# leggedrobotics/raisimLib

Hardware: AMD Instinct MI355X
Metric: env-steps/sec, 4096 ANYmal-C envs flat terrain dt=0.0025 (higher is better)
Workload: dtype f32

## Files before the change

raisimlib_amd/csrc/step_phase_delassus.inc:

```
      const int npw = ncw * (ncw + 1) / 2;
      for (int p0 = 0; p0 < npw; p0 += LPE) {
        const int p = p0 + s;
        const int j = (int)((__builtin_sqrtf(8.0f * (float)p + 1.5f) - 1.0f) * 0.5f);
        const int i = p - ((j * (j + 1)) >> 1);
        if (j < nc) {
          const int bi = __float_as_int(CON[i * kConSlot + 7]), bj = __float_as_int(CON[j * kConSlot + 7]);
          const int li = PARLV[bi] >> 8, lj = PARLV[bj] >> 8;
          int ai[ML], aj[ML];
#if defined(RSB_SPECIALIZED) && RSB_SPEC_DEPTH == 4
          {
            const int4 ri = *reinterpret_cast<const int4*>(ANC + bi * 4), rj = *reinterpret_cast<const int4*>(ANC + bj * 4);
            const int vi[4] = {ri.y, ri.z, ri.w, -1}, vj[4] = {rj.y, rj.z, rj.w, -2};
            RSB_UNROLL for (int l = 0; l < ML; ++l) {
              ai[l] = (l + 1 <= li && l < 3) ? vi[l < 3 ? l : 3] : -1;
              aj[l] = (l + 1 <= lj && l < 3) ? vj[l < 3 ? l : 3] : -2;
            }
          }
#else
          RSB_UNROLL for (int l = 0; l < ML; ++l) {
            ai[l] = (l + 1 <= li) ? ANC[bi * depth + l + 1] : -1;
            aj[l] = (l + 1 <= lj) ? ANC[bj * depth + l + 1] : -2;
          }
#endif
          int lca = 0;
          bool same = true;
          RSB_UNROLL for (int l = 0; l < ML; ++l) { same = same && (ai[l] == aj[l]); lca += same ? 1 : 0; }
          constexpr int CWC = 6 + ML;
          float wi[3][CWC], wj[3][CWC];
          const float* Wi = WC + (3 * i) * cw;
          const float* Wj = WC + (3 * j) * cw;
          RSB_UNROLL for (int rr = 0; rr < 3; ++rr) {
            RSB_UNROLL for (int q4 = 0; q4 < (CWC + 3) / 4; ++q4) {
              float t4[4], u4[4];
              ld4(Wi + rr * cw + 4 * q4, t4); ld4(Wj + rr * cw + 4 * q4, u4);
              RSB_UNROLL for (int e = 0; e < 4; ++e)
                if (4 * q4 + e < CWC) { wi[rr][4 * q4 + e] = t4[e]; wj[rr][4 * q4 + e] = u4[e]; }
            }
          }
          float acc[9];
          RSB_UNROLL for (int q2 = 0; q2 < 9; ++q2) acc[q2] = 0.f;
          RSB_UNROLL for (int e = 0; e < CWC; ++e) {
            const bool on = e < 6 || e < 6 + lca;
            float av[3], bv[3];
            RSB_UNROLL for (int rr = 0; rr < 3; ++rr) { av[rr] = on ? wi[rr][e] : 0.f; bv[rr] = on ? wj[rr][e] : 0.f; }
            RSB_UNROLL for (int rr = 0; rr < 3; ++rr)
              RSB_UNROLL for (int cc = 0; cc < 3; ++cc) acc[3 * rr + cc] += av[rr] * bv[cc];
          }
          if (i == j && CON[i * kConSlot + 15] != 0.f) { acc[0] = 1.f; acc[4] = 1.f; }
          if constexpr (TRI) {
            float* bp = G + tri_off(j, i);
            RSB_UNROLL for (int cc = 0; cc < 3; ++cc) {
              const float row[4] = {acc[cc], acc[3 + cc], acc[6 + cc], 0.f};
              st4(bp + 4 * cc, row);
            }
          } else if constexpr (GROWS) {
            const float B[3][3] = {{acc[0], acc[1], acc[2]}, {acc[3], acc[4], acc[5]}, {acc[6], acc[7], acc[8]}};
            const float Bt[3][3] = {{acc[0], acc[3], acc[6]}, {acc[1], acc[4], acc[7]}, {acc[2], acc[5], acc[8]}};
            gblk_store(G + i * GRP + kGBlock * j, B);
            if (i != j) gblk_store(G + j * GRP + kGBlock * i, Bt);
          } else {
            RSB_UNROLL for (int rr = 0; rr < 3; ++rr)
              RSB_UNROLL for (int cc = 0; cc < 3; ++cc) {
                G[(3 * i + rr) * GS + 4 * j + cc] = acc[3 * rr + cc];
                G[(3 * j + cc) * GS + 4 * i + rr] = acc[3 * rr + cc];
              }
          }
          if (i == j) {
            float gi[12];
            inv3(acc, gi);
            gi[9] = gi[10] = gi[11] = 0.f;
            stv<3>(GINV + 12 * i, gi);
          }
        }
      }
      __syncthreads();
      if constexpr (FIXED) {
        if (s < nc && __float_as_int(CON[s * kConSlot + 11]) < kSelfA) {
          float acc[9], gi[12];
          float* dg = TRI ? G + tri_off(s, s) : (GROWS ? G + s * GRP + kGBlock * s : G + 3 * s * GS + 4 * s);
          const int dgs = TRI ? 4 : GS;
          if constexpr (GROWS) {
            float D[3][3];
            gblk_load(dg, D);
            RSB_UNROLL for (int rr = 0; rr < 3; ++rr) RSB_UNROLL for (int cc = 0; cc < 3; ++cc) acc[3 * rr + cc] = D[rr][cc];
          } else {
            RSB_UNROLL for (int rr = 0; rr < 3; ++rr) {
              float g4[4];
              ld4(dg + rr * dgs, g4);
              acc[3 * rr] = g4[0]; acc[3 * rr + 1] = g4[1]; acc[3 * rr + 2] = g4[2];
            }
          }
          const float reg = kSelfReg * (acc[0] + acc[4] + acc[8]) * (1.0f / 3.0f);
          RSB_UNROLL for (int rr = 0; rr < 3; ++rr) { acc[4 * rr] += reg; dg[GROWS ? g_block_off(rr, rr) : rr * dgs + rr] = acc[4 * rr]; }
          inv3(acc, gi);
          gi[9] = gi[10] = gi[11] = 0.f;
          stv<3>(GINV + 12 * s, gi);
        }
        __syncthreads();
      }
      if (__any(nselfc > 0)) {
        for (int sa = 0; sa + 1 < ncw; ++sa) {
          const bool prim = sa + 1 < nc && (__float_as_int(CON[sa * kConSlot + 11]) & kSelfA) != 0;
          if (!__any(prim)) continue;
          const int sb = sa + 1;
          const float z4[4] = {0.f, 0.f, 0.f, 0.f};
          if constexpr (TRI) {
            if (prim && s < nc) {
              float A[3][3], B[3][3];
              const float Z[3][3] = {{0.f, 0.f, 0.f}, {0.f, 0.f, 0.f}, {0.f, 0.f, 0.f}};
              if (s != sa && s != sb) {
                tri_load(G, sa, s, A); tri_load(G, sb, s, B);
                RSB_UNROLL for (int r = 0; r < 3; ++r) RSB_UNROLL for (int c = 0; c < 3; ++c) A[r][c] += B[r][c];
                tri_store(G, sa, s, A); tri_store(G, sb, s, Z);
              } else if (s == sa) {
                float X[3][3], D[3][3];
                tri_load(G, sa, sa, A); tri_load(G, sb, sb, B); tri_load(G, sb, sa, X);
                RSB_UNROLL for (int r = 0; r < 3; ++r) RSB_UNROLL for (int c = 0; c < 3; ++c) D[r][c] = A[r][c] + B[r][c] + X[r][c] + X[c][r];
                const float ju = SELFT[4 * sa + 3] + SELFT[4 * sb + 3];
                float m4[4];
                ld4(SELFT + 4 * sa, m4);
                RSB_UNROLL for (int rr = 0; rr < 3; ++rr) { CV[3 * sa + rr] += CV[3 * sb + rr]; CV[3 * sb + rr] = 0.f; }
                if (m4[1] > 0.f && ju < -m4[2]) CV[3 * sa + 2] += m4[1] * ju;
                const float reg = (FIXED ? 2.f : 1.f) * kSelfReg * (D[0][0] + D[1][1] + D[2][2]) * (1.0f / 3.0f);
                RSB_UNROLL for (int rr = 0; rr < 3; ++rr) D[rr][rr] += reg;
                const float I3[3][3] = {{1.f, 0.f, 0.f}, {0.f, 1.f, 0.f}, {0.f, 0.f, 1.f}};
                tri_store(G, sa, sa, D); tri_store(G, sb, sa, Z); tri_store(G, sb, sb, I3);
                float acc[9], gi[12];
                RSB_UNROLL for (int r = 0; r < 3; ++r) RSB_UNROLL for (int c = 0; c < 3; ++c) acc[3 * r + c] = D[r][c];
                inv3(acc, gi);
                gi[9] = gi[10] = gi[11] = 0.f;
                stv<3>(GINV + 12 * sa, gi);
                RSB_UNROLL for (int q2 = 0; q2 < 12; ++q2) gi[q2] = 0.f;
                gi[0] = gi[4] = gi[8] = 1.f;
                stv<3>(GINV + 12 * sb, gi);
              }
            }
            __syncthreads();
            continue;
          }
          if (prim && s < nc) {
            if constexpr (GROWS) {
              gblk_add(G + sa * GRP + kGBlock * s, G + sb * GRP + kGBlock * s);
            } else {
              RSB_UNROLL for (int rr = 0; rr < 3; ++rr) {
                float ga[4], gb[4];
                ld4(G + (3 * sa + rr) * GS + 4 * s, ga); ld4(G + (3 * sb + rr) * GS + 4 * s, gb);
                RSB_UNROLL for (int e = 0; e < 4; ++e) ga[e] += gb[e];
                st4(G + (3 * sa + rr) * GS + 4 * s, ga); st4(G + (3 * sb + rr) * GS + 4 * s, z4);
              }
            }
          }
          __syncthreads();
          if constexpr (GROWS) {
            if (prim && s < nc) gblk_add(G + s * GRP + kGBlock * sa, G + s * GRP + kGBlock * sb);
          } else if (prim) {
            for (int r = s; r < 3 * nc; r += LPE) {
              float ga[4], gb[4];
              ld4(G + r * GS + 4 * sa, ga); ld4(G + r * GS + 4 * sb, gb);
              RSB_UNROLL for (int e = 0; e < 4; ++e) ga[e] += gb[e];
              st4(G + r * GS + 4 * sa, ga); st4(G + r * GS + 4 * sb, z4);
            }
          }
          __syncthreads();
          if (prim && s == 0) {
            float m4[4], acc[9], gi[12];
            ld4(SELFT + 4 * sa, m4);
            const float ju = m4[3] + SELFT[4 * sb + 3];
            RSB_UNROLL for (int rr = 0; rr < 3; ++rr) { CV[3 * sa + rr] += CV[3 * sb + rr]; CV[3 * sb + rr] = 0.f; }
            if (m4[1] > 0.f && ju < -m4[2]) CV[3 * sa + 2] += m4[1] * ju;
            if constexpr (GROWS) {
              float D[3][3];
              gblk_load(G + sa * GRP + kGBlock * sa, D);
              RSB_UNROLL for (int rr = 0; rr < 3; ++rr) RSB_UNROLL for (int cc = 0; cc < 3; ++cc) acc[3 * rr + cc] = D[rr][cc];
            } else {
              RSB_UNROLL for (int rr = 0; rr < 3; ++rr) {
                float g4[4];
                ld4(G + (3 * sa + rr) * GS + 4 * sa, g4);
                acc[3 * rr] = g4[0]; acc[3 * rr + 1] = g4[1]; acc[3 * rr + 2] = g4[2];
              }
            }
            const float reg = (FIXED ? 2.f : 1.f) * kSelfReg * (acc[0] + acc[4] + acc[8]) * (1.0f / 3.0f);
            RSB_UNROLL for (int rr = 0; rr < 3; ++rr) { acc[4 * rr] += reg; G[GROWS ? sa * GRP + kGBlock * sa + g_block_off(rr, rr) : (3 * sa + rr) * GS + 4 * sa + rr] = acc[4 * rr]; }
            inv3(acc, gi);
            gi[9] = gi[10] = gi[11] = 0.f;
            stv<3>(GINV + 12 * sa, gi);
            RSB_UNROLL for (int q2 = 0; q2 < 12; ++q2) gi[q2] = 0.f;
            gi[0] = gi[4] = gi[8] = 1.f;
            stv<3>(GINV + 12 * sb, gi);
            RSB_UNROLL for (int rr = 0; rr < 3; ++rr) G[GROWS ? sb * GRP + kGBlock * sb + g_block_off(rr, rr) : (3 * sb + rr) * GS + 4 * sb + rr] = 1.f;
          }
          __syncthreads();
        }
      }
      RSB_STAMP(5)
```

raisimlib_amd/csrc/step_phase_solver.inc:

```
      if (PROF && a.dbg && env == a.dbg_env && env_valid && s == 0) {
        const int n3 = 3 * nc_real;
        a.dbg[0] = (float)nc_real;
        for (int i = 0; i < n3; ++i)
          for (int j = 0; j < n3; ++j)
            a.dbg[1 + i * n3 + j] = GROWS ? G[(i / 3) * GRP + kGBlock * (j / 3) + g_block_off(i % 3, j % 3)] : !TRI ? G[i * GS + 4 * (j / 3) + (j % 3)]
                                          : (i / 3 >= j / 3 ? G[tri_off(i / 3, j / 3) + 4 * (i % 3) + (j % 3)] : G[tri_off(j / 3, i / 3) + 4 * (j % 3) + (i % 3)]);
        for (int i = 0; i < n3; ++i) a.dbg[1 + n3 * n3 + i] = CV[i];
      }
      long long t_gs0 = 0, tz0 = 0; if (PROF && a.prof) t_gs0 = clock64();
      {
        const bool isc = s < nc;
        float Gii[9], Ginv[12], v[3], lam[3] = {0.f, 0.f, 0.f};
        const float* Gmine = GROWS ? G + GRP * min(s, KMAX - 1) : G + 3 * min(s, KMAX - 1) * GS;
        RSB_UNROLL for (int q2 = 0; q2 < 9; ++q2) Gii[q2] = 0.f;
        RSB_UNROLL for (int q2 = 0; q2 < 12; ++q2) Ginv[q2] = 0.f;
        v[0] = v[1] = v[2] = 0.f;
        int gidc = -1 - s;
        if (isc) {
          if constexpr (GROWS) {
            float D[3][3];
            gblk_load(Gmine + kGBlock * s, D);
            RSB_UNROLL for (int rr = 0; rr < 3; ++rr) RSB_UNROLL for (int cc = 0; cc < 3; ++cc) Gii[3 * rr + cc] = D[rr][cc];
          } else {
            RSB_UNROLL for (int rr = 0; rr < 3; ++rr) {
              float g4[4];
              ld4(TRI ? G + tri_off(s, s) + 4 * rr : G + (3 * s + rr) * GS + 4 * s, g4);
              Gii[3 * rr] = g4[0]; Gii[3 * rr + 1] = g4[1]; Gii[3 * rr + 2] = g4[2];
            }
          }
          ldv<3>(GINV + 12 * s, Ginv);
          v[0] = CV[3 * s]; v[1] = CV[3 * s + 1]; v[2] = CV[3 * s + 2];
          const int kb = __float_as_int(CON[s * kConSlot + 7]);
          gidc = ((PARLV[kb] >> 8) >= 1) ? ANC[kb * depth + 1] : 0;
        }
        RSB_ARGS(ag);
        const int mycol = isc ? __float_as_int(CON[s * kConSlot + 11]) : 0;
        if (__any(nselfc > 0)) {
          const bool prim = isc && (mycol & kSelfA) != 0;
          int gidb = __shfl_down(gidc, 1);
          gidb = prim ? gidb : gidc;
          if (isc && (mycol & kSelfB)) { gidc = -1 - s; gidb = gidc; }
          for (int j = 0; j + 1 < ncw; ++j) {
            const int src = (lane & ~(LPE - 1)) | j;
            const int ja = __shfl(gidc, src), jb = __shfl(gidb, src), jp = __shfl(prim ? 1 : 0, src);
            const int lo = min(ja, jb), hi = max(ja, jb);
            if (jp && lo != hi) { gidc = (gidc == hi) ? lo : gidc; gidb = (gidb == hi) ? lo : gidb; }
          }
        }
        float mu = (isc && mycol < ncol) ? COLT[kColSlot * mycol + 5] : RSB_DIM_F32(MU, ag.mu);
        if constexpr (HM2) { if (isc && (mycol & kExtra)) mu = COLT[kColSlot * (mycol & 0xffff) + 5]; }
        if (mycol & kSelfA) mu = SELFT[4 * s];
        const float mu2 = mu * mu;
        const float alpha_init = RSB_DIM_F32(ALPHA_INIT, ag.alpha_init), alpha_min = RSB_DIM_F32(ALPHA_MIN, ag.alpha_min), alpha_decay = RSB_DIM_F32(ALPHA_DECAY, ag.alpha_decay);
        const float threshold = RSB_DIM_F32(THRESHOLD, ag.threshold), stall_factor = RSB_DIM_F32(STALL_FACTOR, ag.stall_factor);
        const int max_iter = RSB_DIM_INT(MAX_ITER, ag.max_iter), section_rounds = RSB_DIM(SECTION_ROUNDS, ag.section_rounds), stall_window = RSB_DIM(STALL_WINDOW, ag.stall_window);
        const int freeze_after = RSB_DIM(FREEZE_AFTER, ag.freeze_after), refine = RSB_DIM(REFINE, ag.refine), multi_fa = RSB_DIM(MULTI_FA, ag.multi_freeze_after);
        SlipCoef sc;
        sc.a0 = Gii[8]; sc.a1 = mu * Gii[6]; sc.a2 = mu * Gii[7];
        sc.n01 = mu * Gii[0]; sc.n02 = mu * Gii[1]; sc.n11 = mu * Gii[3]; sc.n12 = mu * Gii[4];
        sc.n00 = sc.n10 = sc.vn = sc.ls0 = sc.ls1 = 0.f;
#if RSB_PK_SOLVE
        static_assert(!TRI && !COUL, "the packed sweep is the quadruped's energy-rule classes'");
        const f32x2 gcp[3] = {f32x2{Gii[0], Gii[3]}, f32x2{Gii[1], Gii[4]}, f32x2{Gii[2], Gii[5]}};
        const f32x2 gip[3] = {f32x2{Ginv[0], Ginv[3]}, f32x2{Ginv[1], Ginv[4]}, f32x2{Ginv[2], Ginv[5]}};
        const f32x2 mg1 = pk_splat(mu) * gcp[0], mg2 = pk_splat(mu) * gcp[1];
#endif
        float lam_best[3] = {0.f, 0.f, 0.f}, best_rel = 3e38f;
        float sdx = 0.f, sdy = 0.f;
        int sdst = 0;
        float alpha = alpha_init, best_prev = 3e38f, best_cur = 3e38f;
        bool done = (nc == 0), converged = (nc == 0);
        int wcount = 0;

        int gpos = 0, gdw = 1;
        bool light = false;
        bool multi = false;
        int sw_env = stall_window > 0 ? stall_window : -1;
        {
          static_for<0, KMAX / 4>([&](auto bc) {
            constexpr int j0 = 4 * decltype(bc)::value;
            if (j0 < ncw) {
              static_for<0, 4>([&](auto kc2) {
                constexpr int j = j0 + decltype(kc2)::value;
                const int gj = __builtin_amdgcn_update_dpp(0, gidc, 0x150 + j, 0xf, 0xf, true);
                gpos += ((gj == gidc) & (j < s)) ? 1 : 0;
              });
            }
          });
          const int gd = row_max_i32(isc ? gpos + 1 : 1);
          multi = (RSB_DIM(MULTI_DEPTH, ag.multi_depth) > 0) & (gd >= RSB_DIM(MULTI_DEPTH, ag.multi_depth));
          light = multi & (RSB_DIM(MULTI_LIGHT, ag.multi_light) != 0);
          sw_env = multi ? (RSB_DIM(MULTI_SW, ag.multi_stall_window) > 0 ? RSB_DIM(MULTI_SW, ag.multi_stall_window) : -1) : sw_env;
          gdw = env_groups_max<LPE>(gd);
        }
#ifndef RSB_X_AA8
#define RSB_X_AA8 0
#endif
        constexpr bool AA = TRI || RSB_X_AA8;
        const int aa_first = AA ? ag.anderson : 0;
        const float aa_clip = ag.anderson_clip;
        const bool aa_on = AA && multi && aa_first > 0;
        float aa_x[3] = {0.f, 0.f, 0.f}, aa_g[3] = {0.f, 0.f, 0.f}, aa_r[3] = {0.f, 0.f, 0.f};

        const int sm = min(s, KMAX - 1);
        auto coupling = [&](int k, float (&g)[3][4]) {
          if constexpr (TRI) {
            const bool tr = k > sm;
            const float* bp = G + tri_off(tr ? k : sm, tr ? sm : k);
            float t[3][4];
            RSB_UNROLL for (int rr = 0; rr < 3; ++rr) ld4(bp + 4 * rr, t[rr]);
            RSB_UNROLL for (int rr = 0; rr < 3; ++rr) {
              RSB_UNROLL for (int cc = 0; cc < 3; ++cc) g[rr][cc] = tr ? t[cc][rr] : t[rr][cc];
              g[rr][3] = 0.f;
            }
          } else if constexpr (GROWS) {
            float t[3][3];
            gblk_load(Gmine + kGBlock * k, t);
            RSB_UNROLL for (int rr = 0; rr < 3; ++rr) {
              RSB_UNROLL for (int cc = 0; cc < 3; ++cc) g[rr][cc] = t[rr][cc];
              g[rr][3] = 0.f;
            }
          } else {
            RSB_UNROLL for (int rr = 0; rr < 3; ++rr) ld4(Gmine + rr * GS + 4 * k, g[rr]);
          }
        };
#ifndef RSB_X_PK_TRI
#define RSB_X_PK_TRI 1
#endif
        constexpr bool PK = !TRI || RSB_X_PK_TRI;
#ifndef RSB_X_NPK_TRI
#define RSB_X_NPK_TRI 12
#endif
#ifndef RSB_X_NPK_QUAD
#define RSB_X_NPK_QUAD 5
#endif
        constexpr int NPK = TRI ? RSB_X_NPK_TRI : RSB_X_NPK_QUAD;
        typedef float float2v __attribute__((ext_vector_type(2)));
        float g0[PK ? 1 : 4][3][4];
        float g1[PK ? 1 : 4][3][4];
        float2v gp[PK ? NPK : 1][3];
        float gr[PK ? NPK : 1][3];
        if constexpr (PK && !TRI) {
          RSB_UNROLL for (int k = 0; k < NPK; ++k) {
            if (k < 5 || ncw > 5) {
              if constexpr (GROWS) {
                float q0[4], q1[4];
                ld4(Gmine + kGBlock * k, q0); ld4(Gmine + kGBlock * k + 4, q1);
                gp[k][0] = float2v{q0[0], q0[1]}; gp[k][1] = float2v{q0[2], q0[3]}; gp[k][2] = float2v{q1[0], q1[1]};
                gr[k][0] = q1[2]; gr[k][1] = q1[3]; gr[k][2] = Gmine[kGBlock * k + 8];
              } else {
                RSB_UNROLL for (int cc = 0; cc < 3; ++cc) {
                  gp[k][cc] = float2v{Gmine[4 * k + cc], Gmine[GS + 4 * k + cc]};
                  gr[k][cc] = Gmine[2 * GS + 4 * k + cc];
                }
              }
            }
          }
        } else if constexpr (PK) {
          RSB_UNROLL for (int k = 0; k < NPK; ++k) {
            float t[3][4];
            coupling(k, t);
            RSB_UNROLL for (int cc = 0; cc < 3; ++cc) { gp[k][cc] = float2v{t[0][cc], t[1][cc]}; gr[k][cc] = t[2][cc]; }
          }
        } else {
          RSB_UNROLL for (int k = 0; k < 4; ++k) coupling(k, g0[k]);
          RSB_UNROLL for (int k = 0; k < 4; ++k) coupling(4 + k, g1[k]);
        }
        float g2[(KMAX > 8 && !PK) ? 4 : 1][3][4];
        if constexpr (KMAX > 8 && !PK) {
          RSB_UNROLL for (int k = 0; k < 4; ++k) coupling(8 + k, g2[k]);
        }
        float gbuf[2][4][3][4];
        auto load_block = [&](auto bc) {
          constexpr int b = decltype(bc)::value;
          RSB_UNROLL for (int k = 0; k < 4; ++k) coupling(4 * b + k, gbuf[b & 1][k]);
        };
        auto exchange = [&](const float (&x)[3], float& emax) {
          auto one = [&](auto jc) {
            constexpr int j = decltype(jc)::value;
            float l0[3] = {x[0], x[1], x[2]};
            row_bcast_n<j, 3>(l0);
            if constexpr (PK && j < NPK) {
              float2v acc = {v[0], v[1]};
              RSB_UNROLL for (int cc = 0; cc < 3; ++cc) acc = __builtin_elementwise_fma(gp[j][cc], float2v{l0[cc], l0[cc]}, acc);
              v[0] = acc.x; v[1] = acc.y;
              v[2] = fmaf(gr[j][2], l0[2], fmaf(gr[j][1], l0[1], fmaf(gr[j][0], l0[0], v[2])));
            } else if constexpr (PK && !TRI && j < 8) {
              float gt[3][4];
              coupling(j, gt);
              RSB_UNROLL for (int rr = 0; rr < 3; ++rr)
                v[rr] = fmaf(gt[rr][2], l0[2], fmaf(gt[rr][1], l0[1], fmaf(gt[rr][0], l0[0], v[rr])));
            } else {
              const float (&gj)[3][4] = PK ? gbuf[(j / 4) & 1][j & 3] : (j < 4 ? g0[PK ? 0 : (j & 3)] : (j < 8 ? g1[PK ? 0 : (j & 3)] : (j < 12 ? g2[(KMAX > 8 && !PK ? j : 0) & 3] : gbuf[(j / 4) & 1][j & 3])));
              RSB_UNROLL for (int rr = 0; rr < 3; ++rr)
                v[rr] = fmaf(gj[rr][2], l0[2], fmaf(gj[rr][1], l0[1], fmaf(gj[rr][0], l0[0], v[rr])));
            }
            emax = fmaxf(emax, fmaxf(fabsf(l0[0]), fmaxf(fabsf(l0[1]), fabsf(l0[2]))));
          };
          static_for<0, 5>(one);
          {
            if (ncw > 5) {
              one(std::integral_constant<int, 5>{});
              if (ncw > 6) {
                one(std::integral_constant<int, 6>{});
                if (ncw > 7) {
                  one(std::integral_constant<int, 7>{});
                  static_for<2, KMAX / 4>([&](auto bc) {
                    constexpr int b = decltype(bc)::value;
                    if (4 * b < ncw) {
                      if constexpr (b >= 3 || (PK && 4 * b >= NPK)) load_block(bc);
                      static_for<4 * b, 4 * b + 4>(one);
                    }
                  });
                }
              }
            }
          }
        };

        if (has_warm) {
          if (isc) {
            if (mycol < ncol) {
              const float* wr = WARM + 6 * mycol;
              lam[0] = wr[0]; lam[1] = wr[1]; lam[2] = wr[2];
              sdx = wr[3]; sdy = wr[4]; sdst = wr[5] != 0.f ? 3 : 0;
            }
          }
          for (int i = s; i < nwarm; i += LPE) WARM[i] = 0.f;
          if (__any(isc && (lam[0] != 0.f || lam[1] != 0.f || lam[2] != 0.f))) {
            float unused = 0.f;
            exchange(lam, unused);
          }
        }
        if (PROF && pfine) { t_prev = t_gs0; lap(t_setup); }

        auto search_row = [&](int j, const SlipCoef& kc, bool take) {
          if (PROF && a.prof) ++p_search;
          float c12[13] = {kc.a0, kc.a1, kc.a2, kc.n00, kc.n01, kc.n02, kc.n10, kc.n11, kc.n12, kc.vn, kc.ls0, kc.ls1, mu};
          row_bcast_dyn_n<KMAX, 13>(c12, j);
          SlipCoef kb;
          kb.a0 = c12[0]; kb.a1 = c12[1]; kb.a2 = c12[2]; kb.n00 = c12[3]; kb.n01 = c12[4]; kb.n02 = c12[5];
          kb.n10 = c12[6]; kb.n11 = c12[7]; kb.n12 = c12[8]; kb.vn = c12[9]; kb.ls0 = c12[10]; kb.ls1 = c12[11];
          float dxy[2];
          slip_search<LPE, COUL>(kb, c12[12], section_rounds, s, el, c16, s16, DIR16, dxy);
          if (take) { sdx = dxy[0]; sdy = dxy[1]; sdst = 1; }
        };

#if !defined(RSB_X_ALIGN_SWEEP) && defined(RSB_SPECIALIZED)
#define RSB_X_ALIGN_SWEEP 0
#endif
#ifndef RSB_X_ALIGN_SWEEP
#define RSB_X_ALIGN_SWEEP 7
#endif
#ifndef RSB_X_ALIGN_SWEEP_TRI
#define RSB_X_ALIGN_SWEEP_TRI 7
#endif
        asm volatile(".p2align 5");
        static_for<0, (TRI ? RSB_X_ALIGN_SWEEP_TRI : RSB_X_ALIGN_SWEEP)>([&](auto) { asm volatile("s_nop 0"); });
#if RSB_PK_CLASS
        asm volatile("; rsb sweep begin");
#endif
        for (int it = 0; it < max_iter; ++it) {
          const bool lag = multi ? (multi_fa > 0 && it >= multi_fa) : (freeze_after > 0 && it >= freeze_after);
          float err = 0.f;
          float dl_last[3] = {0.f, 0.f, 0.f};
          if constexpr (AA) { aa_x[0] = lam[0]; aa_x[1] = lam[1]; aa_x[2] = lam[2]; }
          for (int kp = 0; kp < gdw; ++kp) {
            const bool mine = isc & !done & (gpos == kp);
            if (PROF && a.prof) ++p_solves;
            float ls[3];
#if RSB_PK_SOLVE
            const f32x2 ls01 = pk_stick(gip, f32x2{v[0], v[1]}, v[2], f32x2{lam[0], lam[1]});
            ls[0] = ls01.x; ls[1] = ls01.y;
            ls[2] = fmaf(-Ginv[8], v[2], fmaf(-Ginv[7], v[1], fmaf(-Ginv[6], v[0], lam[2])));
#else
            RSB_UNROLL for (int rr = 0; rr < 3; ++rr)
              ls[rr] = fmaf(-Ginv[3 * rr + 2], v[2], fmaf(-Ginv[3 * rr + 1], v[1], fmaf(-Ginv[3 * rr], v[0], lam[rr])));
#endif
            const float vexn = fmaf(-Gii[8], lam[2], fmaf(-Gii[7], lam[1], fmaf(-Gii[6], lam[0], v[2])));
            const bool open = vexn > 0.f;
            const bool stick = (!open) & (ls[2] >= 0.f) & (fmaf(ls[1], ls[1], ls[0] * ls[0]) <= (mu2 * ls[2]) * ls[2]);
            const bool slip = (!open) & (!stick);
            const bool usable = (sdst == 1) & (fmaf(sc.a2, sdy, fmaf(sc.a1, sdx, sc.a0)) >= kDenFreeze * sc.a0);
            const bool keep = lag & usable;
            const bool refr = isc & !done & (light ? (kp == 0) : (gpos == kp));
            bool need = refr & slip & !keep;
            const bool lost = mine & slip & !refr & !usable;
            lap(t_rule);
#ifdef RSB_X_NO_NEWTON
            if (false) {
#else
            if (__any(need | lost)) {
#endif
              SlipCoef kc;
              kc = sc;
#if RSB_PK_SOLVE
              SlipCoefPk kp;
              pk_coef(kp, sc.a0, sc.a1, sc.a2, gcp[2], mg1, mg2, pk_vex(gcp, f32x2{v[0], v[1]}, f32x2{lam[0], lam[1]}, lam[2]), vexn, ls01);
              kc = slip_unpack(kp);
#else
              {
                const float vex0 = v[0] - (Gii[0] * lam[0] + Gii[1] * lam[1] + Gii[2] * lam[2]);
                const float vex1 = v[1] - (Gii[3] * lam[0] + Gii[4] * lam[1] + Gii[5] * lam[2]);
                kc.n00 = sc.a0 * vex0 - vexn * Gii[2]; kc.n01 = sc.a1 * vex0 - vexn * sc.n01; kc.n02 = sc.a2 * vex0 - vexn * sc.n02;
                kc.n10 = sc.a0 * vex1 - vexn * Gii[5]; kc.n11 = sc.a1 * vex1 - vexn * sc.n11; kc.n12 = sc.a2 * vex1 - vexn * sc.n12;
                kc.vn = vexn; kc.ls0 = ls[0]; kc.ls1 = ls[1];
              }
#endif
              if (PROF && a.prof) ++p_newton;
              float nx, ny, dstep;
#if RSB_PK_SOLVE
              bool ok = slip_newton_pk(kp, mu, sdx, sdy, nx, ny, dstep) & need & (sdst != 0) & (refine != 0);
#else
              bool ok = slip_newton<COUL>(kc, mu, sdx, sdy, nx, ny, dstep) & need & (sdst != 0) & (refine != 0);
#endif
#ifdef RSB_X_STAMP_BASIN
              lap(t_newt);
#endif
#ifdef RSB_X_NO_BASIN
              if (false) {
#else
              if (it == 0 && !COUL) {
#endif
                const bool chk = ok & (sdst == 3);
                if (__any(chk)) {
                  float ebest;
#ifndef RSB_X_SERIAL_BASIN
                  if (ncw <= 4) {
                    const int row = lane & ~15, q = lane & 3;
                    const int from_owner = (row | ((lane >> 2) & 3)) << 2, from_quad = (row | ((lane & 3) << 2)) << 2;
                    float c13[13] = {kc.a0, kc.a1, kc.a2, kc.n00, kc.n01, kc.n02, kc.n10, kc.n11, kc.n12, kc.vn, kc.ls0, kc.ls1, mu};
                    RSB_UNROLL for (int i = 0; i < 13; ++i) c13[i] = __int_as_float(__builtin_amdgcn_ds_bpermute(from_owner, __float_as_int(c13[i])));
                    SlipCoef kq;
                    kq.a0 = c13[0]; kq.a1 = c13[1]; kq.a2 = c13[2]; kq.n00 = c13[3]; kq.n01 = c13[4]; kq.n02 = c13[5];
                    kq.n10 = c13[6]; kq.n11 = c13[7]; kq.n12 = c13[8]; kq.vn = c13[9]; kq.ls0 = c13[10]; kq.ls1 = c13[11];
                    float e = __int_as_float(0x7f800000);
                    const bool swp = (q & 1) != 0;
                    const unsigned sgx = ((q + 1) & 2) ? 0x80000000u : 0u, sgy = (q & 2) ? 0x80000000u : 0u;
                    RSB_UNROLL for (int i = 0; i < 4; ++i) {
                      const float x = __uint_as_float(__float_as_uint(swp ? kSin16[i] : kCos16[i]) ^ sgx);
                      const float y = __uint_as_float(__float_as_uint(swp ? kCos16[i] : kSin16[i]) ^ sgy);
                      e = fminf(e, slip_E(kq, c13[12], x, y));
                    }
                    e = fminf(e, __int_as_float(__builtin_amdgcn_update_dpp(0, __float_as_int(e), 0xB1, 0xf, 0xf, true)));
                    e = fminf(e, __int_as_float(__builtin_amdgcn_update_dpp(0, __float_as_int(e), 0x4E, 0xf, 0xf, true)));
                    ebest = __int_as_float(__builtin_amdgcn_ds_bpermute(from_quad, __float_as_int(e)));
#ifdef RSB_X_BASIN_VERIFY
                    {
                      float e2 = slip_E(kc, mu, 1.0f, 0.0f);
                      RSB_UNROLL for (int i = 1; i < 16; ++i) e2 = fminf(e2, slip_E(kc, mu, kCos16[i], kSin16[i]));
                      if (chk && __float_as_int(e2) != __float_as_int(ebest)) flag |= 16;
                    }
#endif
                  } else
#endif
                  {
                    SlipCoef ks = kc;
#ifndef RSB_X_SERIAL_BASIN
                    asm volatile("" : "+v"(ks.a0), "+v"(ks.a1), "+v"(ks.a2));
#endif
                    ebest = slip_E(ks, mu, 1.0f, 0.0f);
                    RSB_UNROLL for (int i = 1; i < 16; ++i) ebest = fminf(ebest, slip_E(ks, mu, kCos16[i], kSin16[i]));
                  }
                  ok = ok & !(chk & !(slip_E(kc, mu, nx, ny) <= ebest));
                }
              }
#ifdef RSB_X_STAMP_BASIN
              lap(t_mag);
#endif
              sdx = ok ? nx : sdx; sdy = ok ? ny : sdy; sdst = ok ? 1 : sdst;
              need = (need & !ok) | lost;
              if (__any(need)) {
                for (int j = 0; j < ncw; ++j)
                  if (__any(need && s == j)) search_row(j, kc, need && s == j);
              }
              lap(t_newt);
            }
            const float den = fmaf(sc.a2, sdy, fmaf(sc.a1, sdx, sc.a0));
            const float lnn = -vexn * __builtin_amdgcn_rcpf(fmaxf(den, kDenMin * sc.a0));
            const float ltn = mu * lnn;
            float ln[3];
            float dl[3];
#if RSB_PK_SOLVE
            {
              const f32x2 lt = pk_splat(ltn) * f32x2{sdx, sdy};
              ln[0] = slip ? lt.x : (stick ? ls[0] : 0.f);
              ln[1] = slip ? lt.y : (stick ? ls[1] : 0.f);
              ln[2] = slip ? lnn : (stick ? ls[2] : 0.f);
              const f32x2 l01 = f32x2{lam[0], lam[1]}, df = pk_splat(alpha) * (f32x2{ln[0], ln[1]} - l01);
              dl[0] = mine ? df.x : 0.f; dl[1] = mine ? df.y : 0.f;
              dl[2] = mine ? alpha * (ln[2] - lam[2]) : 0.f;
              const f32x2 ln01 = l01 + f32x2{dl[0], dl[1]};
              lam[0] = ln01.x; lam[1] = ln01.y; lam[2] += dl[2];
            }
#else
            ln[0] = slip ? ltn * sdx : (stick ? ls[0] : 0.f);
            ln[1] = slip ? ltn * sdy : (stick ? ls[1] : 0.f);
            ln[2] = slip ? lnn : (stick ? ls[2] : 0.f);
            RSB_UNROLL for (int rr = 0; rr < 3; ++rr) {
              dl[rr] = mine ? alpha * (ln[rr] - lam[rr]) : 0.f;
              lam[rr] += dl[rr];
            }
#endif
            lap(t_mag);
            if constexpr (AA) {
              if (kp + 1 < gdw) exchange(dl, err);
              else { dl_last[0] = dl[0]; dl_last[1] = dl[1]; dl_last[2] = dl[2]; }
            } else {
              exchange(dl, err);
            }
            lap(t_exch);
          }
          if constexpr (AA)
            err = fmaxf(err, row_max_f32(fmaxf(fabsf(dl_last[0]), fmaxf(fabsf(dl_last[1]), fabsf(dl_last[2])))));
          if (it == 0) sdst = (sdst == 3) ? 0 : sdst;
          const float scale = row_max_f32(isc ? lam[2] : 0.f);
          {
            const bool live = !done;
            iters_used += live ? 1 : 0;
            alpha = fmaxf(alpha * alpha_decay, alpha_min);
            const float denom = scale + kLambdaFloor;
            const bool conv_now = live & (err <= threshold * denom);
            const float rel = err * __builtin_amdgcn_rcpf(denom);
            const bool cont = live & !conv_now;
            const bool better = cont & (rel < best_rel);
            best_rel = better ? rel : best_rel;
            RSB_UNROLL for (int rr = 0; rr < 3; ++rr) lam_best[rr] = better ? lam[rr] : lam_best[rr];
            best_cur = cont ? fminf(best_cur, rel) : best_cur;
            wcount += cont ? 1 : 0;
            const bool wfull = cont & (wcount == sw_env);
            const bool stalled = wfull & (best_cur > stall_factor * best_prev);
            best_prev = wfull ? best_cur : best_prev;
            best_cur = wfull ? 3e38f : best_cur;
            wcount = wfull ? 0 : wcount;
            converged |= conv_now;
            done |= conv_now | stalled;
          }
          lap(t_epi);
          if (!__any(!done)) break;
          if constexpr (AA) {
            if (__any(aa_on & !done)) {
              float rr[3], num = 0.f, den = 0.f;
              RSB_UNROLL for (int q2 = 0; q2 < 3; ++q2) {
                rr[q2] = lam[q2] - aa_x[q2];
                const float dr = rr[q2] - aa_r[q2];
                num = fmaf(rr[q2], dr, num); den = fmaf(dr, dr, den);
              }
              num = row_sum_f32(isc ? num : 0.f); den = row_sum_f32(isc ? den : 0.f);
              if constexpr (LPE > 16) {
                num = __shfl(num, (lane & ~(LPE - 1)) | (lane & 15)); den = __shfl(den, (lane & ~(LPE - 1)) | (lane & 15));
              }
              const bool use = aa_on & !done & (it >= 1) & (it + 1 >= aa_first) & (den > 1e-30f);
              float gam = use ? num / den : 0.f;
              gam = (fabsf(gam) <= aa_clip) ? gam : 0.f;
              float xn[3], dl[3];
              RSB_UNROLL for (int q2 = 0; q2 < 3; ++q2) { xn[q2] = fmaf(-gam, lam[q2] - aa_g[q2], lam[q2]); aa_g[q2] = lam[q2]; aa_r[q2] = rr[q2]; }
              const float t2 = fmaf(xn[1], xn[1], xn[0] * xn[0]), lim = mu * xn[2];
              const float sh = (t2 > lim * lim) ? lim * __builtin_amdgcn_rsqf(t2) : 1.f;
              const bool off = xn[2] <= 0.f;
              xn[0] = off ? 0.f : xn[0] * sh; xn[1] = off ? 0.f : xn[1] * sh; xn[2] = off ? 0.f : xn[2];
              const bool app = isc & (gam != 0.f);
              RSB_UNROLL for (int q2 = 0; q2 < 3; ++q2) { dl[q2] = app ? xn[q2] - lam[q2] : 0.f; lam[q2] += dl[q2]; dl_last[q2] += dl[q2]; }
            }
            float unused = 0.f;
            exchange(dl_last, unused);
          }
        }
#if RSB_PK_CLASS
        asm volatile("; rsb sweep end");
#endif
        if (PROF && pfine) tz0 = t_prev;
        if (!converged) { flag |= 4; lam[0] = lam_best[0]; lam[1] = lam_best[1]; lam[2] = lam_best[2]; }
        if (__any(nselfc > 0)) {
          RSB_UNROLL for (int rr = 0; rr < 3; ++rr) {
            const float up = __shfl_up(lam[rr], 1);
            lam[rr] = (mycol & kSelfB) ? up : lam[rr];
          }
        }
        if (isc) {
          LAM[3 * s] = lam[0]; LAM[3 * s + 1] = lam[1]; LAM[3 * s + 2] = lam[2];
          if (has_warm && mycol < ncol) {
            float* wr = WARM + 6 * mycol;
            wr[0] = lam[0]; wr[1] = lam[1]; wr[2] = lam[2];
            wr[3] = sdst ? sdx : 0.f; wr[4] = sdst ? sdy : 0.f; wr[5] = sdst ? 1.f : 0.f;
          }
        }
        {
          const int sc2 = isc ? s : 0;
          const float* W0 = WC + 3 * sc2 * cw;
          float z0[8], z1[8], z2[8];
          ld4(W0, z0); ld4(W0 + 4, z0 + 4); ld4(W0 + cw, z1); ld4(W0 + cw + 4, z1 + 4); ld4(W0 + 2 * cw, z2); ld4(W0 + 2 * cw + 4, z2 + 4);
          const float l0 = isc ? lam[0] : 0.f, l1 = isc ? lam[1] : 0.f, l2 = isc ? lam[2] : 0.f;
          RSB_UNROLL for (int i = 0; i < 6; ++i) wlam[i] = row_sum_f32(isc ? z0[i] * l0 + z1[i] * l1 + z2[i] * l2 : 0.f);
          if constexpr (LPE > 16) {
            RSB_UNROLL for (int i = 0; i < 6; ++i) wlam[i] = __shfl(wlam[i], (lane & ~(LPE - 1)) | (lane & 15));
          }
#if RSB_FLAT_CLASS
          asm volatile("; rsb scatter begin");
#endif
#if RSB_FLAT_SCATTER
          if (isc) {
            const int bi = __float_as_int(CON[s * kConSlot + 7]);
            int anc[4] = {0, -1, -1, -1};
#if RSB_SPEC_DEPTH == 4
            { const int4 r4 = *reinterpret_cast<const int4*>(ANC + bi * 4); anc[1] = r4.y; anc[2] = r4.z; anc[3] = r4.w; }
#else
            RSB_UNROLL for (int lv = 1; lv < RSB_SPEC_DEPTH; ++lv) anc[lv] = ANC[bi * RSB_SPEC_DEPTH + lv];
#endif
            float* sink = WC + 3 * s * cw + kFlatSink;
            float wl[4] = {0.f, 0.f, 0.f, 0.f};
            RSB_UNROLL for (int lv = 1; lv < RSB_SPEC_DEPTH; ++lv) {
              float w0, w1, w2;
              if (lv < 3) { w0 = z0[5 + lv]; w1 = z1[5 + lv]; w2 = z2[5 + lv]; }
              else { w0 = W0[5 + lv]; w1 = W0[cw + 5 + lv]; w2 = W0[2 * cw + 5 + lv]; }
              wl[lv] = w0 * l0 + w1 * l1 + w2 * l2;
            }
            RSB_UNROLL for (int lv = 1; lv < RSB_SPEC_DEPTH; ++lv) {
              float* dst = (anc[lv] >= 0) ? &WB[anc[lv] + 5] : sink;
              atomicAdd(dst, wl[lv]);
            }
          }
#else
          if (isc) {
            const int bi = __float_as_int(CON[s * kConSlot + 7]);
            int anc[ML + 1];
            RSB_UNROLL for (int lv = 1; lv <= ML; ++lv) anc[lv] = (lv < depth) ? ANC[bi * depth + lv] : -1;
            RSB_UNROLL for (int lv = 1; lv <= ML; ++lv) {
              if (lv < depth) {
                const int b = anc[lv];
                if (b >= 0) {
                  float w0, w1, w2;
                  if (lv < 3) { w0 = z0[5 + lv]; w1 = z1[5 + lv]; w2 = z2[5 + lv]; }
                  else { w0 = W0[5 + lv]; w1 = W0[cw + 5 + lv]; w2 = W0[2 * cw + 5 + lv]; }
                  atomicAdd(&WB[b + 5], w0 * l0 + w1 * l1 + w2 * l2);
                }
              }
            }
          }
#endif
#if RSB_FLAT_CLASS
          asm volatile("; rsb scatter end");
#endif
        }
      }
      __syncthreads();
      if (PROF && pfine) t_end += clock64() - tz0;
      if (PROF && a.prof) { t_gs += clock64() - t_gs0; int itw = iters_used; RSB_UNROLL for (int off = LPE; off < 64; off <<= 1) itw = max(itw, __shfl_xor(itw, off)); p_iters += itw; p_ncw = max(p_ncw, ncw); }
      if (PROF && a.dbg && env == a.dbg_env && env_valid && s == 0) {
        const int n3 = 3 * nc_real;
        for (int i = 0; i < n3; ++i) a.dbg[1 + n3 * n3 + n3 + i] = LAM[i];
      }
```

raisimlib_amd/csrc/step_spec.h:

```cpp
#pragma once

#define RSB_SPEC_FIELDS(X)                                                                                                              \
  X(NB, a.nb) X(NQ, a.nq) X(NV, a.nv) X(DEPTH, a.depth) X(NCOL, a.ncol) X(MAX_KID, a.max_kid) X(FIXED_BASE, (a.fixed_base != 0))      \
  X(N_SELF, a.n_self) X(NSUB, a.nsub) X(KMAX, a.kmax) X(HAS_WARM, (a.warm != nullptr)) X(TERRAIN, a.terrain_type)                      \
  X(EARLY_TERM, (a.early_term != 0)) X(SECTION_ROUNDS, a.section_rounds) X(STALL_WINDOW, a.stall_window) X(FREEZE_AFTER, a.freeze_after) \
  X(REFINE, a.refine) X(MULTI_FA, a.multi_freeze_after) X(MULTI_DEPTH, a.multi_depth) X(MULTI_LIGHT, a.multi_light)                    \
  X(MULTI_SW, a.multi_stall_window) X(CHAIN, (a.chain != 0)) X(MODEL_PITCH, a.L.model_pitch) \
  X(UP_QUADS, (a.chain == 2)) \
  X(MU, rsbk::spec_bits(a.mu)) X(ERP, rsbk::spec_bits(a.erp)) X(ALPHA_INIT, rsbk::spec_bits(a.alpha_init)) X(ALPHA_MIN, rsbk::spec_bits(a.alpha_min)) \
  X(ALPHA_DECAY, rsbk::spec_bits(a.alpha_decay)) X(THRESHOLD, rsbk::spec_bits(a.threshold)) X(STALL_FACTOR, rsbk::spec_bits(a.stall_factor)) \
  X(MAX_ITER, a.max_iter)

#ifdef RSB_SPECIALIZED
#define RSB_DIM(NAME, expr) (RSB_SPEC_##NAME)
#else
#define RSB_DIM(NAME, expr) (expr)
#endif

namespace rsbk {
constexpr int spec_bits(float f) { return __builtin_bit_cast(int, f); }
constexpr float spec_f32(int bits) { return __builtin_bit_cast(float, bits); }
}
#if defined(RSB_SPECIALIZED) && !defined(RSB_X_NO_SPEC_CONSTS)
#define RSB_SPEC_CONSTS 1
#define RSB_DIM_F32(NAME, expr) (rsbk::spec_f32((int)(RSB_SPEC_##NAME)))
#define RSB_DIM_INT(NAME, expr) ((int)(RSB_SPEC_##NAME))
#else
#define RSB_SPEC_CONSTS 0
#define RSB_DIM_F32(NAME, expr) (expr)
#define RSB_DIM_INT(NAME, expr) (expr)
#endif

#if defined(RSB_SPECIALIZED) && RSB_SPEC_UP_QUADS && !defined(RSB_X_NO_UP_QUADS)
#define RSB_UP_QUADS 1
#if !RSB_SPEC_CHAIN
#error "RSB_SPEC_UP_QUADS: the quad form of the up pass is for consecutively numbered chains (RSB_SPEC_CHAIN)"
#endif
#else
#define RSB_UP_QUADS 0
#endif

#if RSB_UP_QUADS && !defined(RSB_X_NO_DOWN_QUADS)
#define RSB_DOWN_QUADS 1
#else
#define RSB_DOWN_QUADS 0
#endif

#if RSB_DOWN_QUADS && !defined(RSB_X_NO_SEAM_CARRY)
#define RSB_SEAM_CARRY 1
#else
#define RSB_SEAM_CARRY 0
#endif
#if RSB_SEAM_CARRY && !defined(RSB_X_NO_SEAM_JOINTS)
#define RSB_SEAM_JOINTS 1
#else
#define RSB_SEAM_JOINTS 0
#endif
#if RSB_SEAM_CARRY && !defined(RSB_X_NO_SEAM_BASE)
#define RSB_SEAM_BASE 1
#else
#define RSB_SEAM_BASE 0
#endif
#if RSB_SEAM_CARRY && !defined(RSB_X_NO_SEAM_LOADS)
#define RSB_SEAM_LOADS 1
#else
#define RSB_SEAM_LOADS 0
#endif

#if defined(RSB_SPECIALIZED) && defined(RSB_I_CL) && (RSB_I_CL) == 64 && (RSB_I_LPE) == 16 && (RSB_I_KMAX) == 8 && RSB_SPEC_NQ > 16 && RSB_SPEC_NQ <= 32 && \
    RSB_SPEC_NQ + RSB_SPEC_NV > 32 && RSB_SPEC_NQ + RSB_SPEC_NV <= 48 && !defined(RSB_X_NO_LEAN_SEAM)
#define RSB_LEAN_SEAM 1
#else
#define RSB_LEAN_SEAM 0
#endif

#if defined(RSB_SPECIALIZED) && defined(RSB_I_LPE) && (RSB_I_LPE) == 16 && (RSB_I_KMAX) <= 8 && (RSB_I_ML) <= 4 && RSB_SPEC_DEPTH >= 2 && RSB_SPEC_DEPTH <= 4 && \
    RSB_SPEC_DEPTH <= (RSB_I_ML) && ((6 + RSB_SPEC_DEPTH - 1 + 3) & ~3) > 6 + RSB_SPEC_DEPTH - 1
#define RSB_FLAT_CLASS 1
#else
#define RSB_FLAT_CLASS 0
#endif
#if RSB_FLAT_CLASS && !defined(RSB_X_NO_FLAT_CONTACT)
#define RSB_FLAT_CONTACT 1
#else
#define RSB_FLAT_CONTACT 0
#endif
#if RSB_FLAT_CONTACT && !defined(RSB_X_NO_FLAT_COLUMNS)
#define RSB_FLAT_COLUMNS 1
#else
#define RSB_FLAT_COLUMNS 0
#endif
#if RSB_FLAT_CONTACT && !defined(RSB_X_NO_FLAT_SCATTER)
#define RSB_FLAT_SCATTER 1
#else
#define RSB_FLAT_SCATTER 0
#endif
#if RSB_FLAT_CLASS
namespace rsbk {
constexpr int kFlatCw = (6 + RSB_SPEC_DEPTH - 1 + 3) & ~3, kFlatSink = kFlatCw - 1;
static_assert(kFlatSink >= 6 + RSB_SPEC_DEPTH - 1 && kFlatSink < kFlatCw, "flat contact form: the sink must be a padding entry of the column");
}
#endif

#if defined(RSB_SPECIALIZED) && defined(RSB_I_LPE) && (RSB_I_LPE) == 16 && (RSB_I_KMAX) <= 8 && !((RSB_I_CL) & 32)
#define RSB_PK_CLASS 1
#else
#define RSB_PK_CLASS 0
#endif
#if RSB_PK_CLASS && !defined(RSB_X_NO_PK_SOLVE)
#define RSB_PK_SOLVE 1
#else
#define RSB_PK_SOLVE 0
#endif

namespace rsbk {
#define RSB_SPEC_COUNT_ONE(NAME, expr) +1
constexpr int kSpecFields = 0 RSB_SPEC_FIELDS(RSB_SPEC_COUNT_ONE);
#undef RSB_SPEC_COUNT_ONE
}
```

Baseline: 374.6 million.

## Hoist and batch solver setup loads and restructure end-phase writeback for flat class

```diff
diff --git a/raisimlib_amd/csrc/step_phase_delassus.inc b/raisimlib_amd/csrc/step_phase_delassus.inc
--- a/raisimlib_amd/csrc/step_phase_delassus.inc
+++ b/raisimlib_amd/csrc/step_phase_delassus.inc
@@ -25,7 +25,11 @@
           int lca = 0;
           bool same = true;
           RSB_UNROLL for (int l = 0; l < ML; ++l) { same = same && (ai[l] == aj[l]); lca += same ? 1 : 0; }
+#if RSB_FLAT_SETUP_HEAD
+          constexpr int CWC = 6 + RSB_SPEC_DEPTH - 1;
+#else
           constexpr int CWC = 6 + ML;
+#endif
           float wi[3][CWC], wj[3][CWC];
           const float* Wi = WC + (3 * i) * cw;
           const float* Wj = WC + (3 * j) * cw;
diff --git a/raisimlib_amd/csrc/step_phase_solver.inc b/raisimlib_amd/csrc/step_phase_solver.inc
--- a/raisimlib_amd/csrc/step_phase_solver.inc
+++ b/raisimlib_amd/csrc/step_phase_solver.inc
@@ -15,6 +15,39 @@
         RSB_UNROLL for (int q2 = 0; q2 < 9; ++q2) Gii[q2] = 0.f;
         RSB_UNROLL for (int q2 = 0; q2 < 12; ++q2) Ginv[q2] = 0.f;
         v[0] = v[1] = v[2] = 0.f;
+#if RSB_FLAT_CLASS
+        asm volatile("; rsb setup begin");
+#endif
+#if RSB_FLAT_SETUP_HEAD
+        static_assert(GROWS && !TRI, "flat set-up: the row-block layout of the quadruped classes");
+        const int sq = min(s, KMAX - 1);
+        float fq0[5][4], fq1[5][4], fq2[5], fc4[4], fc8[4];
+        {
+          float D[3][3];
+          gblk_load(Gmine + kGBlock * sq, D);
+          ldv<3>(GINV + 12 * sq, Ginv);
+          v[0] = CV[3 * sq]; v[1] = CV[3 * sq + 1]; v[2] = CV[3 * sq + 2];
+          ld4(CON + sq * kConSlot + 4, fc4); ld4(CON + sq * kConSlot + 8, fc8);
+          RSB_UNROLL for (int k = 0; k < 5; ++k) { ld4(Gmine + kGBlock * k, fq0[k]); ld4(Gmine + kGBlock * k + 4, fq1[k]); fq2[k] = Gmine[kGBlock * k + 8]; }
+          RSB_UNROLL for (int rr = 0; rr < 3; ++rr) RSB_UNROLL for (int cc = 0; cc < 3; ++cc) Gii[3 * rr + cc] = D[rr][cc];
+        }
+        const int kb = isc ? __float_as_int(fc4[3]) : 0;
+        const int mycol = isc ? __float_as_int(fc8[3]) : 0;
+        const int fci = min(mycol & 0xffff, ncol - 1);
+        const int fpl = PARLV[kb];
+        int fanc[4] = {0, -1, -1, -1};
+#if RSB_SPEC_DEPTH == 4
+        { const int4 r4 = *reinterpret_cast<const int4*>(ANC + kb * 4); fanc[1] = r4.y; fanc[2] = r4.z; fanc[3] = r4.w; }
+#else
+        RSB_UNROLL for (int lv = 1; lv < RSB_SPEC_DEPTH; ++lv) fanc[lv] = ANC[kb * RSB_SPEC_DEPTH + lv];
+#endif
+        const float fmu = COLT[kColSlot * fci + 5];
+        float fwr[6] = {0.f, 0.f, 0.f, 0.f, 0.f, 0.f};
+        if (has_warm) { RSB_UNROLL for (int i = 0; i < 6; ++i) fwr[i] = WARM[6 * fci + i]; }
+        __builtin_amdgcn_sched_barrier(0);
+        int gidc = isc ? (((fpl >> 8) >= 1) ? fanc[1] : 0) : -1 - s;
+        float fsmu = 0.f;
+#else
         int gidc = -1 - s;
         if (isc) {
           if constexpr (GROWS) {
@@ -33,9 +66,15 @@
           const int kb = __float_as_int(CON[s * kConSlot + 7]);
           gidc = ((PARLV[kb] >> 8) >= 1) ? ANC[kb * depth + 1] : 0;
         }
+#endif
         RSB_ARGS(ag);
+#if !RSB_FLAT_SETUP_HEAD
         const int mycol = isc ? __float_as_int(CON[s * kConSlot + 11]) : 0;
+#endif
         if (__any(nselfc > 0)) {
+#if RSB_FLAT_SETUP_HEAD
+          fsmu = SELFT[4 * sq];
+#endif
           const bool prim = isc && (mycol & kSelfA) != 0;
           int gidb = __shfl_down(gidc, 1);
           gidb = prim ? gidb : gidc;
@@ -47,9 +86,15 @@
             if (jp && lo != hi) { gidc = (gidc == hi) ? lo : gidc; gidb = (gidb == hi) ? lo : gidb; }
           }
         }
+#if RSB_FLAT_SETUP_HEAD
+        float mu = (isc && mycol < ncol) ? fmu : RSB_DIM_F32(MU, ag.mu);
+        if constexpr (HM2) mu = (isc && (mycol & kExtra)) ? fmu : mu;
+        mu = (mycol & kSelfA) ? fsmu : mu;
+#else
         float mu = (isc && mycol < ncol) ? COLT[kColSlot * mycol + 5] : RSB_DIM_F32(MU, ag.mu);
         if constexpr (HM2) { if (isc && (mycol & kExtra)) mu = COLT[kColSlot * (mycol & 0xffff) + 5]; }
         if (mycol & kSelfA) mu = SELFT[4 * s];
+#endif
         const float mu2 = mu * mu;
         const float alpha_init = RSB_DIM_F32(ALPHA_INIT, ag.alpha_init), alpha_min = RSB_DIM_F32(ALPHA_MIN, ag.alpha_min), alpha_decay = RSB_DIM_F32(ALPHA_DECAY, ag.alpha_decay);
         const float threshold = RSB_DIM_F32(THRESHOLD, ag.threshold), stall_factor = RSB_DIM_F32(STALL_FACTOR, ag.stall_factor);
@@ -142,6 +187,13 @@
         float gr[PK ? NPK : 1][3];
         if constexpr (PK && !TRI) {
           RSB_UNROLL for (int k = 0; k < NPK; ++k) {
+#if RSB_FLAT_SETUP_HEAD
+            static_assert(NPK >= 5, "flat set-up: batch A reads the five blocks of the exchange's straight part");
+            if (k < 5) {
+              gp[k][0] = float2v{fq0[k][0], fq0[k][1]}; gp[k][1] = float2v{fq0[k][2], fq0[k][3]}; gp[k][2] = float2v{fq1[k][0], fq1[k][1]};
+              gr[k][0] = fq1[k][2]; gr[k][1] = fq1[k][3]; gr[k][2] = fq2[k < 5 ? k : 0];
+            } else
+#endif
             if (k < 5 || ncw > 5) {
               if constexpr (GROWS) {
                 float q0[4], q1[4];
@@ -219,6 +271,17 @@
         };
 
         if (has_warm) {
+#if RSB_FLAT_SETUP_HEAD
+          {
+            const bool wok = isc && mycol < ncol;
+            lam[0] = wok ? fwr[0] : 0.f; lam[1] = wok ? fwr[1] : 0.f; lam[2] = wok ? fwr[2] : 0.f;
+            sdx = wok ? fwr[3] : 0.f; sdy = wok ? fwr[4] : 0.f; sdst = (wok && fwr[5] != 0.f) ? 3 : 0;
+          }
+          {
+            constexpr int kNw = 6 * RSB_SPEC_NCOL, kTrips = (kNw + LPE - 1) / LPE;
+            RSB_UNROLL for (int t = 0; t < kTrips; ++t) WARM[(LPE * (t + 1) <= kNw) ? s + LPE * t : min(s + LPE * t, kNw - 1)] = 0.f;
+          }
+#else
           if (isc) {
             if (mycol < ncol) {
               const float* wr = WARM + 6 * mycol;
@@ -227,12 +290,20 @@
             }
           }
           for (int i = s; i < nwarm; i += LPE) WARM[i] = 0.f;
+#endif
+#if RSB_FLAT_SETUP_HEAD
+          if (__any(isc & ((lam[0] != 0.f) | (lam[1] != 0.f) | (lam[2] != 0.f)))) {
+#else
           if (__any(isc && (lam[0] != 0.f || lam[1] != 0.f || lam[2] != 0.f))) {
+#endif
             float unused = 0.f;
             exchange(lam, unused);
           }
         }
         if (PROF && pfine) { t_prev = t_gs0; lap(t_setup); }
+#if RSB_FLAT_CLASS
+        asm volatile("; rsb setup end");
+#endif
 
         auto search_row = [&](int j, const SlipCoef& kc, bool take) {
           if (PROF && a.prof) ++p_search;
@@ -469,14 +540,23 @@
 #if RSB_PK_CLASS
         asm volatile("; rsb sweep end");
 #endif
+#if RSB_FLAT_CLASS
+        asm volatile("; rsb solver end begin");
+#endif
         if (PROF && pfine) tz0 = t_prev;
+#if RSB_FLAT_SETUP_END
+        flag |= converged ? 0 : 4;
+        lam[0] = converged ? lam[0] : lam_best[0]; lam[1] = converged ? lam[1] : lam_best[1]; lam[2] = converged ? lam[2] : lam_best[2];
+#else
         if (!converged) { flag |= 4; lam[0] = lam_best[0]; lam[1] = lam_best[1]; lam[2] = lam_best[2]; }
+#endif
         if (__any(nselfc > 0)) {
           RSB_UNROLL for (int rr = 0; rr < 3; ++rr) {
             const float up = __shfl_up(lam[rr], 1);
             lam[rr] = (mycol & kSelfB) ? up : lam[rr];
           }
         }
+#if !RSB_FLAT_SETUP_END
         if (isc) {
           LAM[3 * s] = lam[0]; LAM[3 * s + 1] = lam[1]; LAM[3 * s + 2] = lam[2];
           if (has_warm && mycol < ncol) {
@@ -485,20 +565,60 @@
             wr[3] = sdst ? sdx : 0.f; wr[4] = sdst ? sdy : 0.f; wr[5] = sdst ? 1.f : 0.f;
           }
         }
+#endif
         {
           const int sc2 = isc ? s : 0;
           const float* W0 = WC + 3 * sc2 * cw;
           float z0[8], z1[8], z2[8];
           ld4(W0, z0); ld4(W0 + 4, z0 + 4); ld4(W0 + cw, z1); ld4(W0 + cw + 4, z1 + 4); ld4(W0 + 2 * cw, z2); ld4(W0 + 2 * cw + 4, z2 + 4);
+#if RSB_FLAT_SETUP_END
+          float zt[3][RSB_SPEC_DEPTH > 3 ? RSB_SPEC_DEPTH - 3 : 1];
+          RSB_UNROLL for (int lv = 3; lv < RSB_SPEC_DEPTH; ++lv) { zt[0][lv - 3] = W0[5 + lv]; zt[1][lv - 3] = W0[cw + 5 + lv]; zt[2][lv - 3] = W0[2 * cw + 5 + lv]; }
+          RSB_UNROLL for (int i = 0; i < 8; ++i) asm volatile("" : "+v"(z0[i]), "+v"(z1[i]), "+v"(z2[i]));
+#if !RSB_FLAT_SETUP_HEAD
+          int fanc[4] = {0, -1, -1, -1};
+          {
+            const int bi = isc ? __float_as_int(CON[sc2 * kConSlot + 7]) : 0;
+#if RSB_SPEC_DEPTH == 4
+            const int4 r4 = *reinterpret_cast<const int4*>(ANC + bi * 4); fanc[1] = r4.y; fanc[2] = r4.z; fanc[3] = r4.w;
+#else
+            RSB_UNROLL for (int lv = 1; lv < RSB_SPEC_DEPTH; ++lv) fanc[lv] = ANC[bi * RSB_SPEC_DEPTH + lv];
+#endif
+          }
+#endif
+#endif
           const float l0 = isc ? lam[0] : 0.f, l1 = isc ? lam[1] : 0.f, l2 = isc ? lam[2] : 0.f;
           RSB_UNROLL for (int i = 0; i < 6; ++i) wlam[i] = row_sum_f32(isc ? z0[i] * l0 + z1[i] * l1 + z2[i] * l2 : 0.f);
           if constexpr (LPE > 16) {
             RSB_UNROLL for (int i = 0; i < 6; ++i) wlam[i] = __shfl(wlam[i], (lane & ~(LPE - 1)) | (lane & 15));
           }
-#if RSB_FLAT_CLASS
+#if RSB_FLAT_CLASS && !RSB_FLAT_SETUP_END
           asm volatile("; rsb scatter begin");
 #endif
-#if RSB_FLAT_SCATTER
+#if RSB_FLAT_SETUP_END
+          if (isc) {
+            LAM[3 * s] = lam[0]; LAM[3 * s + 1] = lam[1]; LAM[3 * s + 2] = lam[2];
+            if (has_warm && mycol < ncol) {
+              float* wr = WARM + 6 * mycol;
+              wr[0] = lam[0]; wr[1] = lam[1]; wr[2] = lam[2];
+              wr[3] = sdst ? sdx : 0.f; wr[4] = sdst ? sdy : 0.f; wr[5] = sdst ? 1.f : 0.f;
+            }
+            asm volatile("; rsb scatter begin");
+            float* sink = WC + 3 * s * cw + kFlatSink;
+            float wl[4] = {0.f, 0.f, 0.f, 0.f};
+            RSB_UNROLL for (int lv = 1; lv < RSB_SPEC_DEPTH; ++lv) {
+              float w0, w1, w2;
+              if (lv < 3) { w0 = z0[5 + lv]; w1 = z1[5 + lv]; w2 = z2[5 + lv]; }
+              else { w0 = zt[0][lv < 3 ? 0 : lv - 3]; w1 = zt[1][lv < 3 ? 0 : lv - 3]; w2 = zt[2][lv < 3 ? 0 : lv - 3]; }
+              wl[lv] = w0 * lam[0] + w1 * lam[1] + w2 * lam[2];
+            }
+            RSB_UNROLL for (int lv = 1; lv < RSB_SPEC_DEPTH; ++lv) {
+              float* dst = (fanc[lv] >= 0) ? &WB[fanc[lv] + 5] : sink;
+              atomicAdd(dst, wl[lv]);
+            }
+            asm volatile("; rsb scatter end");
+          }
+#elif RSB_FLAT_SCATTER
           if (isc) {
             const int bi = __float_as_int(CON[s * kConSlot + 7]);
             int anc[4] = {0, -1, -1, -1};
@@ -538,10 +658,13 @@
             }
           }
 #endif
+#if RSB_FLAT_CLASS && !RSB_FLAT_SETUP_END
+          asm volatile("; rsb scatter end");
+#endif
+        }
 #if RSB_FLAT_CLASS
-          asm volatile("; rsb scatter end");
-#endif
-        }
+        asm volatile("; rsb solver end end");
+#endif
       }
       __syncthreads();
       if (PROF && pfine) t_end += clock64() - tz0;
diff --git a/raisimlib_amd/csrc/step_spec.h b/raisimlib_amd/csrc/step_spec.h
--- a/raisimlib_amd/csrc/step_spec.h
+++ b/raisimlib_amd/csrc/step_spec.h
@@ -102,6 +102,22 @@
 }
 #endif
 
+#if RSB_FLAT_CLASS && !((RSB_I_CL) & (32 | 1)) && !defined(RSB_X_G_SQUARE) && !defined(RSB_X_NO_FLAT_SETUP)
+#define RSB_FLAT_SETUP 1
+#else
+#define RSB_FLAT_SETUP 0
+#endif
+#if RSB_FLAT_SETUP && !defined(RSB_X_NO_FLAT_SETUP_HEAD)
+#define RSB_FLAT_SETUP_HEAD 1
+#else
+#define RSB_FLAT_SETUP_HEAD 0
+#endif
+#if RSB_FLAT_SETUP && RSB_FLAT_SCATTER && !defined(RSB_X_NO_FLAT_SETUP_END)
+#define RSB_FLAT_SETUP_END 1
+#else
+#define RSB_FLAT_SETUP_END 0
+#endif
+
 #if defined(RSB_SPECIALIZED) && defined(RSB_I_LPE) && (RSB_I_LPE) == 16 && (RSB_I_KMAX) <= 8 && !((RSB_I_CL) & 32)
 #define RSB_PK_CLASS 1
 #else
```

New measurement: 390.5 million (median of 6 runs). +4.2%, better.
